# ChenRocks/UNITER

Measured on NVIDIA H100. Metric: uniter_base_encoder_fwd_bwd_samples_per_sec, higher is better.
Workload: dtype bf16

## Files before the change

uniter_b200/csrc/attn.cu:

```cuda
#include "common.h"
#include "ptx.cuh"
#include "wgmma.cuh"

namespace ub {

constexpr int ATT_D = 64;
constexpr int ATT_BM = 128;
constexpr int ATT_BN = 128;
constexpr int ATT_TILE = ATT_BM * ATT_D * 2;
constexpr int ATT_MAXSEQ = 512;
constexpr int ATT_THREADS = 256;

struct AttnParams {
  const int* cu_seqlens;
  int B, H, nheads, T;
  void* ctx;
  float* lse;
  float scale;
  uint32_t drop_thr16;
  float drop_inv_keep;
  uint32_t seed_lo, seed_hi, stream_lo, stream_hi;
  const void* dctx;
  void* dqkv;
  float* dbias;
  const unsigned long long* rng_dev;
};


__device__ __forceinline__ void frag_colsum64_atomic(const float (&d)[32], bool ok0, bool ok1, float* dst,
                                                     int lane) {
#pragma unroll
  for (int jj = 0; jj < 8; ++jj) {
#pragma unroll
    for (int t = 0; t < 2; ++t) {
      float x = (ok0 ? d[4 * jj + t] : 0.f) + (ok1 ? d[4 * jj + 2 + t] : 0.f);
      x += __shfl_xor_sync(0xffffffffu, x, 4);
      x += __shfl_xor_sync(0xffffffffu, x, 8);
      x += __shfl_xor_sync(0xffffffffu, x, 16);
      if (lane < 4) atomicAdd(dst + 8 * jj + 2 * lane + t, x);
    }
  }
}

__device__ __forceinline__ void frag_colsum64_warp(const float (&d)[32], bool ok0, bool ok1, float* dst, int lane) {
#pragma unroll
  for (int jj = 0; jj < 8; ++jj) {
#pragma unroll
    for (int t = 0; t < 2; ++t) {
      float x = (ok0 ? d[4 * jj + t] : 0.f) + (ok1 ? d[4 * jj + 2 + t] : 0.f);
      x += __shfl_xor_sync(0xffffffffu, x, 4);
      x += __shfl_xor_sync(0xffffffffu, x, 8);
      x += __shfl_xor_sync(0xffffffffu, x, 16);
      if (lane < 4) dst[8 * jj + 2 * lane + t] += x;
    }
  }
}

template <bool kBF16>
__device__ __forceinline__ void store_frag_row(void* out_row, const float (&d)[32], int e, int q4, float mul) {
  uint32_t* o = reinterpret_cast<uint32_t*>(out_row);
#pragma unroll
  for (int jj = 0; jj < 8; ++jj)
    o[(8 * jj + 2 * q4) >> 1] = Elem<kBF16>::pack(d[4 * jj + 2 * e] * mul, d[4 * jj + 2 * e + 1] * mul);
}

__device__ __forceinline__ uint64_t attn_drop_group(int bh, int q, int key8) {
  return ((static_cast<uint64_t>(bh) * ATT_MAXSEQ + q) * ATT_MAXSEQ + key8) >> 3;
}

__device__ __forceinline__ void quad_drop_words(const DropoutRng& rng, int bh, int q, int key_base, int jb,
                                                int lane, uint32_t (&w)[4]) {
  const int q4 = lane & 3;
  const uint4 r = rng.draw8(attn_drop_group(bh, q, key_base + 8 * (4 * jb + q4)));
  uint32_t got[4];
#pragma unroll
  for (int k = 0; k < 4; ++k) {
    const int sw = (q4 - k) & 3;
    const uint32_t v = sw == 0 ? r.x : (sw == 1 ? r.y : (sw == 2 ? r.z : r.w));
    got[k] = __shfl_sync(0xffffffffu, v, (lane & ~3) | ((q4 + k) & 3));
  }
#pragma unroll
  for (int t = 0; t < 4; ++t) {
    const int k = (t - q4) & 3;
    w[t] = k == 0 ? got[0] : (k == 1 ? got[1] : (k == 2 ? got[2] : got[3]));
  }
}

__device__ __forceinline__ uint32_t rand16_half(uint32_t w, int t) { return t ? (w >> 16) : (w & 0xFFFFu); }

__device__ __forceinline__ void st_swz128_u32(uint8_t* base, int r, int col, uint32_t v) {
  const int slab = col >> 6;
  const int chunk = (col & 63) >> 3;
  uint8_t* p = base + slab * ATT_TILE + r * 128 + ((chunk ^ (r & 7)) << 4) + (col & 7) * 2;
  *reinterpret_cast<uint32_t*>(p) = v;
}

template <bool kBF16>
__device__ __forceinline__ void row_delta_lse(const AttnParams& p, int seq0, int head, int row, bool ok, int q4,
                                              float& delta, float& lse2) {
  using T16 = typename Elem<kBF16>::T;
  float d = 0.f;
  lse2 = 0.f;
  if (ok) {
    const size_t off = static_cast<size_t>(seq0 + row) * p.H + head * ATT_D + 16 * q4;
    const uint4* g_do = reinterpret_cast<const uint4*>(reinterpret_cast<const T16*>(p.dctx) + off);
    const uint4* g_o = reinterpret_cast<const uint4*>(reinterpret_cast<const T16*>(p.ctx) + off);
#pragma unroll
    for (int v = 0; v < 2; ++v) {
      const uint4 a = __ldg(g_do + v), o = __ldg(g_o + v);
      float2 x, y;
      x = Elem<kBF16>::unpack(a.x); y = Elem<kBF16>::unpack(o.x); d += x.x * y.x + x.y * y.y;
      x = Elem<kBF16>::unpack(a.y); y = Elem<kBF16>::unpack(o.y); d += x.x * y.x + x.y * y.y;
      x = Elem<kBF16>::unpack(a.z); y = Elem<kBF16>::unpack(o.z); d += x.x * y.x + x.y * y.y;
      x = Elem<kBF16>::unpack(a.w); y = Elem<kBF16>::unpack(o.w); d += x.x * y.x + x.y * y.y;
    }
    lse2 = p.lse[static_cast<size_t>(head) * p.T + seq0 + row] * 1.4426950408889634f;
  }
  d += __shfl_xor_sync(0xffffffffu, d, 1);
  d += __shfl_xor_sync(0xffffffffu, d, 2);
  delta = d;
}

constexpr int SH_TILE = 64 * ATT_D * 2;
constexpr int SH_THREADS = 128;
constexpr int SH_MAXSEQ = 128;

__device__ __forceinline__ void wg_sync() { asm volatile("bar.sync 1, 128;" ::: "memory"); }

__device__ __forceinline__ int seq_blocks(const int* cu, int b) { return min((cu[b + 1] - cu[b] + 63) >> 6, 2); }

struct ShortSched {
  const int* cu;
  int B, nheads, h, b;
  long long start, hi;

  __device__ bool valid() const { return h < nheads && start < hi; }
  __device__ int blocks() const { return seq_blocks(cu, b); }

  __device__ void init(const int* cu_, int B_, int nheads_, int lane) {
    cu = cu_; B = B_; nheads = nheads_;
    h = nheads; start = hi = 0;
    int wb = 0;
    for (int b0 = 0; b0 < B; b0 += 32) {
      int c = b0 + lane < B ? seq_blocks(cu, b0 + lane) : 0;
      c *= c;
#pragma unroll
      for (int d = 16; d >= 1; d >>= 1) c += __shfl_xor_sync(0xffffffffu, c, d);
      wb += c;
    }
    if (wb == 0) return;
    const long long W = static_cast<long long>(nheads) * wb;
    const long long lo = W * blockIdx.x / gridDim.x;
    hi = W * (blockIdx.x + 1) / gridDim.x;
    if (lo >= hi) return;
    const int hh = static_cast<int>(lo / wb);
    const long long r = lo - static_cast<long long>(hh) * wb;
    int pref = 0;
    for (int b0 = 0; b0 < B; b0 += 32) {
      int c = b0 + lane < B ? seq_blocks(cu, b0 + lane) : 0;
      c *= c;
      int incl = c;
#pragma unroll
      for (int d = 1; d < 32; d <<= 1) {
        const int t = __shfl_up_sync(0xffffffffu, incl, d);
        if (lane >= d) incl += t;
      }
      const int excl = pref + incl - c;
      const unsigned m = __ballot_sync(0xffffffffu, b0 + lane < B && excl >= r);
      if (m) {
        const int L = __ffs(m) - 1;
        h = hh;
        b = b0 + L;
        start = static_cast<long long>(hh) * wb + __shfl_sync(0xffffffffu, excl, L);
        skip_empty();
        return;
      }
      pref += __shfl_sync(0xffffffffu, incl, 31);
    }
    h = hh + 1;
    b = 0;
    start = static_cast<long long>(h) * wb;
    skip_empty();
  }
  __device__ void step() {
    const int nb = blocks();
    start += nb * nb;
    if (++b == B) { b = 0; ++h; }
  }
  __device__ void skip_empty() {
    while (valid() && cu[b + 1] == cu[b]) step();
  }
  __device__ void next() { step(); skip_empty(); }
};

template <bool kBF16, int NB>
__device__ __forceinline__ void attn_fwd_short_rows(const AttnParams& p, uint32_t uQ, uint32_t uK, uint32_t uV,
                                                    int qb, int S, int seq0, int head, int bh,
                                                    const DropoutRng& rng, int warp, int lane) {
  const int q4 = lane & 3;
  const float c = p.scale * 1.4426950408889634f;
  int qrow[2];
#pragma unroll
  for (int e = 0; e < 2; ++e) qrow[e] = 64 * qb + 16 * warp + (lane >> 2) + 8 * e;

  float s[NB][32];
  wgmma_fence();
#pragma unroll
  for (int kb = 0; kb < NB; ++kb)
#pragma unroll
    for (int k = 0; k < ATT_D / 16; ++k)
      Wgmma<64, kBF16, 0, 0>::ss(s[kb], gmma_desc(uQ + qb * SH_TILE + k * 32, 16, 1024),
                                 gmma_desc(uK + kb * SH_TILE + k * 32, 16, 1024), k != 0);
  wgmma_commit();
  wgmma_wait<0>();

  float m[2] = {-INFINITY, -INFINITY}, l[2] = {0.f, 0.f};
#pragma unroll
  for (int kb = 0; kb < NB; ++kb)
#pragma unroll
    for (int i = 0; i < 32; ++i) {
      const int key = 64 * kb + 8 * (i >> 2) + 2 * q4 + (i & 1);
      if (key < S) m[(i >> 1) & 1] = fmaxf(m[(i >> 1) & 1], s[kb][i]);
    }
#pragma unroll
  for (int e = 0; e < 2; ++e) {
    m[e] = fmaxf(m[e], __shfl_xor_sync(0xffffffffu, m[e], 1));
    m[e] = fmaxf(m[e], __shfl_xor_sync(0xffffffffu, m[e], 2));
  }
  const float mc[2] = {m[0] * c, m[1] * c};

#pragma unroll
  for (int kb = 0; kb < NB; ++kb) {
#pragma unroll
    for (int jb = 0; jb < 2; ++jb) {
      uint32_t dw[2][4];
#pragma unroll
      for (int e = 0; e < 2; ++e)
        if (p.drop_thr16) quad_drop_words(rng, bh, qrow[e], 64 * kb, jb, lane, dw[e]);
#pragma unroll
      for (int jq = 0; jq < 4; ++jq) {
        const int jj = 4 * jb + jq;
#pragma unroll
        for (int e = 0; e < 2; ++e) {
#pragma unroll
          for (int t = 0; t < 2; ++t) {
            const int i = 4 * jj + 2 * e + t;
            const int key = 64 * kb + 8 * jj + 2 * q4 + t;
            float pv = key < S ? ex2_approx(fmaf(s[kb][i], c, -mc[e])) : 0.f;
            l[e] += pv;
            if (p.drop_thr16) {
              const float pr = Elem<kBF16>::to_f(Elem<kBF16>::from_f(pv));
              pv = (rand16_half(dw[e][jq], t) < p.drop_thr16) ? 0.f : pr * p.drop_inv_keep;
            }
            s[kb][i] = pv;
          }
        }
      }
    }
  }

  float o[32];
  wgmma_fence();
#pragma unroll
  for (int kb = 0; kb < NB; ++kb)
#pragma unroll
    for (int kk = 0; kk < 4; ++kk) {
      const uint32_t a[4] = {Elem<kBF16>::pack(s[kb][8 * kk + 0], s[kb][8 * kk + 1]),
                             Elem<kBF16>::pack(s[kb][8 * kk + 2], s[kb][8 * kk + 3]),
                             Elem<kBF16>::pack(s[kb][8 * kk + 4], s[kb][8 * kk + 5]),
                             Elem<kBF16>::pack(s[kb][8 * kk + 6], s[kb][8 * kk + 7])};
      Wgmma<64, kBF16, 0, 1>::rs(o, a, gmma_desc(uV + kb * SH_TILE + kk * 2048, 8192, 1024), (kb | kk) != 0);
    }
  wgmma_commit();
  wgmma_wait<0>();

#pragma unroll
  for (int e = 0; e < 2; ++e) {
    l[e] += __shfl_xor_sync(0xffffffffu, l[e], 1);
    l[e] += __shfl_xor_sync(0xffffffffu, l[e], 2);
    if (qrow[e] >= S) continue;
    if (q4 == 0) p.lse[static_cast<size_t>(head) * p.T + seq0 + qrow[e]] = m[e] * p.scale + logf(l[e]);
    typename Elem<kBF16>::T* out = reinterpret_cast<typename Elem<kBF16>::T*>(p.ctx) +
                                   static_cast<size_t>(seq0 + qrow[e]) * p.H + head * ATT_D;
    store_frag_row<kBF16>(out, o, e, q4, 1.f / l[e]);
  }
}

template <bool kBF16>
__global__ void __launch_bounds__(SH_THREADS, 2)
attn_fwd_short_kernel(const __grid_constant__ CUtensorMap tmQKV64, const AttnParams p) {
  pdl_launch_dependents();
  pdl_wait();
  extern __shared__ __align__(1024) uint8_t smem_raw[];
  uint8_t* smem = smem_raw + ((1024u - (smem_u32(smem_raw) & 1023u)) & 1023u);
  uint8_t* sQ = smem;
  uint8_t* sK = smem + 2 * SH_TILE;
  uint8_t* sV = smem + 4 * SH_TILE;
  uint64_t* bar = reinterpret_cast<uint64_t*>(smem + 6 * SH_TILE);

  const int tid = threadIdx.x, warp = tid >> 5, lane = tid & 31;
  if (tid == 0) {
    tma_prefetch_desc(&tmQKV64);
    mbar_init(&bar[0], 1);
    mbar_init(&bar[1], 1);
    fence_barrier_init();
  }
  wg_sync();
  uint32_t rs0 = p.stream_lo, rs1 = p.stream_hi;
  if (p.drop_thr16) rng_add_dev_offset(p.rng_dev, rs0, rs1);
  DropoutRng rng;
  rng.k0 = p.seed_lo; rng.k1 = p.seed_hi; rng.s0 = rs0; rng.s1 = rs1;

  auto load = [&](const ShortSched& it, int slot) {
    const int seq0 = p.cu_seqlens[it.b], nb = it.blocks(), col = it.h * ATT_D;
    mbar_expect_tx(&bar[slot], nb * 3 * SH_TILE);
    for (int r = 0; r < nb; ++r) {
      const int o = (slot + r) * SH_TILE;
      tma_load_2d(sQ + o, &tmQKV64, &bar[slot], col, seq0 + 64 * r);
      tma_load_2d(sK + o, &tmQKV64, &bar[slot], p.H + col, seq0 + 64 * r);
      tma_load_2d(sV + o, &tmQKV64, &bar[slot], 2 * p.H + col, seq0 + 64 * r);
    }
  };

  ShortSched it;
  it.init(p.cu_seqlens, p.B, p.nheads, lane);
  if (it.valid() && tid == 0) load(it, 0);
  int slot = 0;
  uint32_t ph = 0;
  while (it.valid()) {
    ShortSched nx = it;
    nx.next();
    const int seq0 = p.cu_seqlens[it.b], S = p.cu_seqlens[it.b + 1] - seq0, nb = it.blocks();
    const bool pre = nx.valid() && nb == 1 && nx.blocks() == 1;
    const int nslot = pre ? slot ^ 1 : 0;
    if (pre && tid == 0) load(nx, nslot);
    mbar_wait(&bar[slot], (ph >> slot) & 1);
    ph ^= 1u << slot;
    const uint32_t uQ = smem_u32(sQ + slot * SH_TILE), uK = smem_u32(sK + slot * SH_TILE),
                   uV = smem_u32(sV + slot * SH_TILE);
    const int bh = it.b * p.nheads + it.h;
    if (nb == 1) {
      attn_fwd_short_rows<kBF16, 1>(p, uQ, uK, uV, 0, S, seq0, it.h, bh, rng, warp, lane);
    } else {
#pragma unroll 1
      for (int qb = 0; qb < 2; ++qb)
        attn_fwd_short_rows<kBF16, 2>(p, uQ, uK, uV, qb, S, seq0, it.h, bh, rng, warp, lane);
    }
    wg_sync();
    if (nx.valid() && !pre && tid == 0) load(nx, 0);
    it = nx;
    slot = nslot;
  }
}

constexpr int SH_FWD_SMEM = 6 * SH_TILE + 16 + 1024;

template <bool kBF16, int NB>
__device__ __forceinline__ void dq_block(float (&dq)[32], uint32_t uDS, uint32_t uK, int qb) {
  wgmma_fence();
#pragma unroll
  for (int kk = 0; kk < 4 * NB; ++kk)
    Wgmma<64, kBF16, 0, 1>::ss(dq, gmma_desc(uDS + (qb * NB + (kk >> 2)) * SH_TILE + (kk & 3) * 32, 16, 1024),
                               gmma_desc(uK + kk * 2048, 8192, 1024), kk != 0);
  wgmma_commit();
  wgmma_wait<0>();
}

template <bool kBF16, bool kBias = true>
__global__ void __launch_bounds__(SH_THREADS, 2)
attn_bwd_short_kernel(const __grid_constant__ CUtensorMap tmQKV64, const __grid_constant__ CUtensorMap tmDO64,
                      const AttnParams p) {
  using T16 = typename Elem<kBF16>::T;
  pdl_launch_dependents();
  pdl_wait();
  extern __shared__ __align__(1024) uint8_t smem_raw[];
  __shared__ float sBias[4][3 * ATT_D];
  uint8_t* smem = smem_raw + ((1024u - (smem_u32(smem_raw) & 1023u)) & 1023u);
  uint8_t* sQ = smem;
  uint8_t* sK = smem + 2 * SH_TILE;
  uint8_t* sV = smem + 4 * SH_TILE;
  uint8_t* sdO = smem + 6 * SH_TILE;
  uint8_t* sP = smem + 8 * SH_TILE;
  uint8_t* sDS = smem + 9 * SH_TILE;
  uint64_t* bar = reinterpret_cast<uint64_t*>(smem + 13 * SH_TILE);

  const int tid = threadIdx.x, warp = tid >> 5, lane = tid & 31, q4 = lane & 3;
  if (tid == 0) {
    tma_prefetch_desc(&tmQKV64);
    tma_prefetch_desc(&tmDO64);
    mbar_init(&bar[0], 1);
    mbar_init(&bar[1], 1);
    fence_barrier_init();
  }
  for (int i = tid; i < 4 * 3 * ATT_D; i += SH_THREADS) (&sBias[0][0])[i] = 0.f;
  wg_sync();
  uint32_t rs0 = p.stream_lo, rs1 = p.stream_hi;
  if (p.drop_thr16) rng_add_dev_offset(p.rng_dev, rs0, rs1);
  DropoutRng rng;
  rng.k0 = p.seed_lo; rng.k1 = p.seed_hi; rng.s0 = rs0; rng.s1 = rs1;
  const float c = p.scale * 1.4426950408889634f;
  int r_loc[2];
#pragma unroll
  for (int e = 0; e < 2; ++e) r_loc[e] = 16 * warp + (lane >> 2) + 8 * e;
  const uint32_t uP = smem_u32(sP), uDS = smem_u32(sDS);

  auto load = [&](const ShortSched& it, int slot) {
    const int seq0 = p.cu_seqlens[it.b], nb = it.blocks(), col = it.h * ATT_D;
    mbar_expect_tx(&bar[slot], nb * 4 * SH_TILE);
    for (int r = 0; r < nb; ++r) {
      const int o = (slot + r) * SH_TILE;
      tma_load_2d(sQ + o, &tmQKV64, &bar[slot], col, seq0 + 64 * r);
      tma_load_2d(sK + o, &tmQKV64, &bar[slot], p.H + col, seq0 + 64 * r);
      tma_load_2d(sV + o, &tmQKV64, &bar[slot], 2 * p.H + col, seq0 + 64 * r);
      tma_load_2d(sdO + o, &tmDO64, &bar[slot], col, seq0 + 64 * r);
    }
  };

  ShortSched it;
  it.init(p.cu_seqlens, p.B, p.nheads, lane);
  if (it.valid() && tid == 0) load(it, 0);
  int slot = 0;
  uint32_t ph = 0;
  while (it.valid()) {
    ShortSched nx = it;
    nx.next();
    const int seq0 = p.cu_seqlens[it.b], S = p.cu_seqlens[it.b + 1] - seq0, nb = it.blocks();
    const int head = it.h, bh = it.b * p.nheads + head;
    const bool pre = nx.valid() && nb == 1 && nx.blocks() == 1;
    const int nslot = pre ? slot ^ 1 : 0;
    if (pre && tid == 0) load(nx, nslot);
    mbar_wait(&bar[slot], (ph >> slot) & 1);
    ph ^= 1u << slot;
    const uint32_t uQ = smem_u32(sQ + slot * SH_TILE), udO = smem_u32(sdO + slot * SH_TILE),
                   uK = smem_u32(sK + slot * SH_TILE), uV = smem_u32(sV + slot * SH_TILE);

    for (int kb = 0; kb < nb; ++kb) {
      float dv[32], dk[32];
      for (int qb = 0; qb < nb; ++qb) {
        int qrow[2];
        bool q_ok[2];
        float delta[2], lse2[2];
#pragma unroll
        for (int e = 0; e < 2; ++e) {
          qrow[e] = 64 * qb + r_loc[e];
          q_ok[e] = qrow[e] < S;
          row_delta_lse<kBF16>(p, seq0, head, qrow[e], q_ok[e], q4, delta[e], lse2[e]);
        }
        float s[32], dp[32];
        wgmma_fence();
#pragma unroll
        for (int k = 0; k < ATT_D / 16; ++k)
          Wgmma<64, kBF16, 0, 0>::ss(s, gmma_desc(uQ + qb * SH_TILE + k * 32, 16, 1024),
                                     gmma_desc(uK + kb * SH_TILE + k * 32, 16, 1024), k != 0);
#pragma unroll
        for (int k = 0; k < ATT_D / 16; ++k)
          Wgmma<64, kBF16, 0, 0>::ss(dp, gmma_desc(udO + qb * SH_TILE + k * 32, 16, 1024),
                                     gmma_desc(uV + kb * SH_TILE + k * 32, 16, 1024), k != 0);
        wgmma_commit();
        wgmma_wait<0>();

        uint8_t* dsTile = sDS + (qb * nb + kb) * SH_TILE;
#pragma unroll
        for (int jb = 0; jb < 2; ++jb) {
          uint32_t dw[2][4];
#pragma unroll
          for (int e = 0; e < 2; ++e)
            if (p.drop_thr16) quad_drop_words(rng, bh, qrow[e], 64 * kb, jb, lane, dw[e]);
#pragma unroll
          for (int jq = 0; jq < 4; ++jq) {
            const int jj = 4 * jb + jq;
#pragma unroll
            for (int e = 0; e < 2; ++e) {
              float pd[2], ds[2];
#pragma unroll
              for (int t = 0; t < 2; ++t) {
                const int idx = 4 * jj + 2 * e + t;
                const bool ok = q_ok[e] && 64 * kb + 8 * jj + 2 * q4 + t < S;
                float pr = ok ? ex2_approx(fmaf(s[idx], c, -lse2[e])) : 0.f;
                pr = Elem<kBF16>::to_f(Elem<kBF16>::from_f(pr));
                float dpv = dp[idx];
                float pdv = pr;
                if (p.drop_thr16) {
                  const bool drop = rand16_half(dw[e][jq], t) < p.drop_thr16;
                  pdv = drop ? 0.f : pr * p.drop_inv_keep;
                  dpv = drop ? 0.f : dpv * p.drop_inv_keep;
                }
                pd[t] = pdv;
                ds[t] = ok ? pr * (dpv - delta[e]) * p.scale : 0.f;
              }
              st_swz128_u32(sP, r_loc[e], 8 * jj + 2 * q4, Elem<kBF16>::pack(pd[0], pd[1]));
              st_swz128_u32(dsTile, r_loc[e], 8 * jj + 2 * q4, Elem<kBF16>::pack(ds[0], ds[1]));
            }
          }
        }
        fence_proxy_async_smem();
        wg_sync();

        const uint32_t uDSt = smem_u32(dsTile);
        wgmma_fence();
#pragma unroll
        for (int kk = 0; kk < 4; ++kk)
          Wgmma<64, kBF16, 1, 1>::ss(dv, gmma_desc(uP + kk * 2048, SH_TILE, 1024),
                                     gmma_desc(udO + qb * SH_TILE + kk * 2048, 8192, 1024), (qb | kk) != 0);
#pragma unroll
        for (int kk = 0; kk < 4; ++kk)
          Wgmma<64, kBF16, 1, 1>::ss(dk, gmma_desc(uDSt + kk * 2048, SH_TILE, 1024),
                                     gmma_desc(uQ + qb * SH_TILE + kk * 2048, 8192, 1024), (qb | kk) != 0);
        wgmma_commit();
        wgmma_wait<0>();
        wg_sync();
      }
      int key[2];
      bool k_ok[2];
#pragma unroll
      for (int e = 0; e < 2; ++e) {
        key[e] = 64 * kb + r_loc[e];
        k_ok[e] = key[e] < S;
      }
      if (kBias && p.dbias) {
        frag_colsum64_warp(dk, k_ok[0], k_ok[1], sBias[warp] + ATT_D, lane);
        frag_colsum64_warp(dv, k_ok[0], k_ok[1], sBias[warp] + 2 * ATT_D, lane);
      }
#pragma unroll
      for (int e = 0; e < 2; ++e) {
        if (!k_ok[e]) continue;
        T16* outk = reinterpret_cast<T16*>(p.dqkv) + static_cast<size_t>(seq0 + key[e]) * (3 * p.H) + p.H +
                    head * ATT_D;
        store_frag_row<kBF16>(outk, dk, e, q4, 1.f);
        store_frag_row<kBF16>(outk + p.H, dv, e, q4, 1.f);
      }
    }

    for (int qb = 0; qb < nb; ++qb) {
      float dq[32];
      if (nb == 1) dq_block<kBF16, 1>(dq, uDS, uK, 0);
      else dq_block<kBF16, 2>(dq, uDS, uK, qb);
      bool q_ok[2];
#pragma unroll
      for (int e = 0; e < 2; ++e) q_ok[e] = 64 * qb + r_loc[e] < S;
      if (kBias && p.dbias) frag_colsum64_warp(dq, q_ok[0], q_ok[1], sBias[warp], lane);
#pragma unroll
      for (int e = 0; e < 2; ++e)
        if (q_ok[e])
          store_frag_row<kBF16>(reinterpret_cast<T16*>(p.dqkv) + static_cast<size_t>(seq0 + 64 * qb + r_loc[e]) *
                                                                       (3 * p.H) + head * ATT_D,
                                dq, e, q4, 1.f);
    }
    wg_sync();
    if (nx.valid() && !pre && tid == 0) load(nx, 0);
    if (kBias && p.dbias && (!nx.valid() || nx.h != head)) {
      for (int i = tid; i < 3 * ATT_D; i += SH_THREADS) {
        atomicAdd(p.dbias + (i >> 6) * p.H + head * ATT_D + (i & 63),
                  (sBias[0][i] + sBias[1][i]) + (sBias[2][i] + sBias[3][i]));
        sBias[0][i] = sBias[1][i] = sBias[2][i] = sBias[3][i] = 0.f;
      }
    }
    it = nx;
    slot = nslot;
  }
}

constexpr int SH_BWD_SMEM = 13 * SH_TILE + 16 + 1024;

template <bool kBF16>
__device__ __forceinline__ void qk_block(float (&s)[64], uint32_t sA, uint32_t sB, int wg) {
#pragma unroll
  for (int k = 0; k < ATT_D / 16; ++k)
    Wgmma<128, kBF16, 0, 0>::ss(s, gmma_desc(sA + wg * (64 * 128) + k * 32, 16, 1024),
                                gmma_desc(sB + k * 32, 16, 1024), k != 0);
}

template <bool kBF16>
__global__ void __launch_bounds__(ATT_THREADS, 1)
attn_fwd_kernel(const __grid_constant__ CUtensorMap tmQKV, const AttnParams p) {
  pdl_launch_dependents();
  pdl_wait();
  const int b = blockIdx.z, qt = blockIdx.x;
  const int seq0 = p.cu_seqlens[b];
  const int S = p.cu_seqlens[b + 1] - seq0;
  if (qt * ATT_BM >= S) return;
  const int head = blockIdx.y;
  const int nkv = (S + ATT_BN - 1) / ATT_BN;
  uint32_t rs0 = p.stream_lo, rs1 = p.stream_hi;
  if (p.drop_thr16) rng_add_dev_offset(p.rng_dev, rs0, rs1);

  extern __shared__ __align__(1024) uint8_t smem_raw[];
  uint8_t* smem = smem_raw + ((1024u - (smem_u32(smem_raw) & 1023u)) & 1023u);
  uint8_t* sQ = smem;
  uint8_t* sK = smem + ATT_TILE;
  uint8_t* sV = smem + 2 * ATT_TILE;
  uint64_t* bar_load = reinterpret_cast<uint64_t*>(smem + 3 * ATT_TILE);

  const int tid = threadIdx.x, warp = tid >> 5, lane = tid & 31;
  const int wg = warp >> 2, q4 = lane & 3;
  if (tid == 0) {
    tma_prefetch_desc(&tmQKV);
    mbar_init(bar_load, 1);
    fence_barrier_init();
  }
  __syncthreads();

  int qrow[2];
  bool q_ok[2];
#pragma unroll
  for (int e = 0; e < 2; ++e) {
    qrow[e] = qt * ATT_BM + 64 * wg + 16 * (warp & 3) + (lane >> 2) + 8 * e;
    q_ok[e] = qrow[e] < S;
  }
  const int bh = b * p.nheads + head;
  const float c = p.scale * 1.4426950408889634f;
  const uint32_t uQ = smem_u32(sQ), uK = smem_u32(sK), uV = smem_u32(sV);
  uint32_t ph_load = 0;
  float s[64];

  float m[2] = {-INFINITY, -INFINITY}, l[2] = {0.f, 0.f};
  for (int j = 0; j < nkv; ++j) {
    const int kv_len = min(ATT_BN, S - j * ATT_BN);
    if (tid == 0) {
      const bool with_v = (nkv == 1);
      mbar_expect_tx(bar_load, (j == 0 ? ATT_TILE : 0) + ATT_TILE + (with_v ? ATT_TILE : 0));
      if (j == 0) tma_load_2d(sQ, &tmQKV, bar_load, head * ATT_D, seq0 + qt * ATT_BM);
      tma_load_2d(sK, &tmQKV, bar_load, p.H + head * ATT_D, seq0 + j * ATT_BN);
      if (with_v) tma_load_2d(sV, &tmQKV, bar_load, 2 * p.H + head * ATT_D, seq0 + j * ATT_BN);
    }
    mbar_wait(bar_load, ph_load);
    ph_load ^= 1;
    wgmma_fence();
    qk_block<kBF16>(s, uQ, uK, wg);
    wgmma_commit();
    wgmma_wait<0>();
#pragma unroll
    for (int i = 0; i < 64; ++i) {
      const int key = 8 * (i >> 2) + 2 * q4 + (i & 1);
      if (key < kv_len) m[(i >> 1) & 1] = fmaxf(m[(i >> 1) & 1], s[i]);
    }
    if (nkv > 1) __syncthreads();
  }
#pragma unroll
  for (int e = 0; e < 2; ++e) {
    m[e] = fmaxf(m[e], __shfl_xor_sync(0xffffffffu, m[e], 1));
    m[e] = fmaxf(m[e], __shfl_xor_sync(0xffffffffu, m[e], 2));
  }
  const float mc[2] = {m[0] * c, m[1] * c};

  float o[32];
#pragma unroll
  for (int i = 0; i < 32; ++i) o[i] = 0.f;
  for (int j = 0; j < nkv; ++j) {
    const int kv_len = min(ATT_BN, S - j * ATT_BN);
    if (nkv > 1) {
      if (tid == 0) {
        mbar_expect_tx(bar_load, 2 * ATT_TILE);
        tma_load_2d(sK, &tmQKV, bar_load, p.H + head * ATT_D, seq0 + j * ATT_BN);
        tma_load_2d(sV, &tmQKV, bar_load, 2 * p.H + head * ATT_D, seq0 + j * ATT_BN);
      }
      mbar_wait(bar_load, ph_load);
      ph_load ^= 1;
      wgmma_fence();
      qk_block<kBF16>(s, uQ, uK, wg);
      wgmma_commit();
      wgmma_wait<0>();
    }
    DropoutRng rng;
    rng.k0 = p.seed_lo; rng.k1 = p.seed_hi; rng.s0 = rs0; rng.s1 = rs1;
#pragma unroll
    for (int jb = 0; jb < 4; ++jb) {
      uint32_t dw[2][4];
#pragma unroll
      for (int e = 0; e < 2; ++e)
        if (p.drop_thr16) quad_drop_words(rng, bh, qrow[e], j * ATT_BN, jb, lane, dw[e]);
#pragma unroll
      for (int jq = 0; jq < 4; ++jq) {
        const int jj = 4 * jb + jq;
#pragma unroll
        for (int e = 0; e < 2; ++e) {
#pragma unroll
          for (int t = 0; t < 2; ++t) {
            const int i = 4 * jj + 2 * e + t;
            const int key = 8 * jj + 2 * q4 + t;
            float pv = key < kv_len ? ex2_approx(fmaf(s[i], c, -mc[e])) : 0.f;
            l[e] += pv;
            if (p.drop_thr16) {
              const float pr = Elem<kBF16>::to_f(Elem<kBF16>::from_f(pv));
              pv = (rand16_half(dw[e][jq], t) < p.drop_thr16) ? 0.f : pr * p.drop_inv_keep;
            }
            s[i] = pv;
          }
        }
      }
    }
    wgmma_fence();
#pragma unroll
    for (int kk = 0; kk < ATT_BN / 16; ++kk) {
      const uint32_t a[4] = {Elem<kBF16>::pack(s[8 * kk + 0], s[8 * kk + 1]),
                             Elem<kBF16>::pack(s[8 * kk + 2], s[8 * kk + 3]),
                             Elem<kBF16>::pack(s[8 * kk + 4], s[8 * kk + 5]),
                             Elem<kBF16>::pack(s[8 * kk + 6], s[8 * kk + 7])};
      Wgmma<64, kBF16, 0, 1>::rs(o, a, gmma_desc(uV + kk * 2048, 8192, 1024), (j | kk) != 0);
    }
    wgmma_commit();
    wgmma_wait<0>();
    if (nkv > 1) __syncthreads();
  }

#pragma unroll
  for (int e = 0; e < 2; ++e) {
    l[e] += __shfl_xor_sync(0xffffffffu, l[e], 1);
    l[e] += __shfl_xor_sync(0xffffffffu, l[e], 2);
    if (!q_ok[e]) continue;
    if (q4 == 0) p.lse[static_cast<size_t>(head) * p.T + seq0 + qrow[e]] = m[e] * p.scale + logf(l[e]);
    typename Elem<kBF16>::T* out = reinterpret_cast<typename Elem<kBF16>::T*>(p.ctx) +
                                   static_cast<size_t>(seq0 + qrow[e]) * p.H + head * ATT_D;
    store_frag_row<kBF16>(out, o, e, q4, 1.f / l[e]);
  }
}

constexpr int ATT_FWD_SMEM = 3 * ATT_TILE + 64 + 1024;

template <bool kBF16>
__global__ void __launch_bounds__(ATT_THREADS, 1)
attn_bwd_kernel(const __grid_constant__ CUtensorMap tmQKV, const __grid_constant__ CUtensorMap tmDO,
                const AttnParams p, float* dq_accum) {
  using T16 = typename Elem<kBF16>::T;
  pdl_launch_dependents();
  pdl_wait();
  const int b = blockIdx.z, j = blockIdx.x;
  const int seq0 = p.cu_seqlens[b];
  const int S = p.cu_seqlens[b + 1] - seq0;
  if (j * ATT_BN >= S) return;
  const int head = blockIdx.y;
  const int nq = (S + ATT_BM - 1) / ATT_BM;
  const int nkv = (S + ATT_BN - 1) / ATT_BN;
  uint32_t rs0 = p.stream_lo, rs1 = p.stream_hi;
  if (p.drop_thr16) rng_add_dev_offset(p.rng_dev, rs0, rs1);
  const int kv_len = min(ATT_BN, S - j * ATT_BN);

  extern __shared__ __align__(1024) uint8_t smem_raw[];
  uint8_t* smem = smem_raw + ((1024u - (smem_u32(smem_raw) & 1023u)) & 1023u);
  uint8_t* sQ = smem;
  uint8_t* sdO = smem + ATT_TILE;
  uint8_t* sK = smem + 2 * ATT_TILE;
  uint8_t* sV = smem + 3 * ATT_TILE;
  uint8_t* sP = smem + 4 * ATT_TILE;
  uint8_t* sDS = smem + 6 * ATT_TILE;
  uint64_t* bar_load = reinterpret_cast<uint64_t*>(smem + 8 * ATT_TILE);

  const int tid = threadIdx.x, warp = tid >> 5, lane = tid & 31;
  const int wg = warp >> 2, q4 = lane & 3;
  if (tid == 0) {
    tma_prefetch_desc(&tmQKV);
    tma_prefetch_desc(&tmDO);
    mbar_init(bar_load, 1);
    fence_barrier_init();
  }
  __syncthreads();
  int r_loc[2];
#pragma unroll
  for (int e = 0; e < 2; ++e) r_loc[e] = 64 * wg + 16 * (warp & 3) + (lane >> 2) + 8 * e;
  const int bh = b * p.nheads + head;
  const float c = p.scale * 1.4426950408889634f;
  const uint32_t uQ = smem_u32(sQ), udO = smem_u32(sdO), uK = smem_u32(sK), uV = smem_u32(sV);
  const uint32_t uP = smem_u32(sP), uDS = smem_u32(sDS);
  uint32_t ph_load = 0;
  float dv[32], dk[32];
#pragma unroll
  for (int i = 0; i < 32; ++i) { dv[i] = 0.f; dk[i] = 0.f; }

  for (int i = 0; i < nq; ++i) {
    int qrow[2];
    bool q_ok[2];
#pragma unroll
    for (int e = 0; e < 2; ++e) {
      qrow[e] = i * ATT_BM + r_loc[e];
      q_ok[e] = qrow[e] < S;
    }
    if (tid == 0) {
      mbar_expect_tx(bar_load, (i == 0 ? 4 : 2) * ATT_TILE);
      tma_load_2d(sQ, &tmQKV, bar_load, head * ATT_D, seq0 + i * ATT_BM);
      tma_load_2d(sdO, &tmDO, bar_load, head * ATT_D, seq0 + i * ATT_BM);
      if (i == 0) {
        tma_load_2d(sK, &tmQKV, bar_load, p.H + head * ATT_D, seq0 + j * ATT_BN);
        tma_load_2d(sV, &tmQKV, bar_load, 2 * p.H + head * ATT_D, seq0 + j * ATT_BN);
      }
    }

    float delta[2], lse2[2];
#pragma unroll
    for (int e = 0; e < 2; ++e) row_delta_lse<kBF16>(p, seq0, head, qrow[e], q_ok[e], q4, delta[e], lse2[e]);

    mbar_wait(bar_load, ph_load);
    ph_load ^= 1;
    float s[64], dp[64];
    wgmma_fence();
    qk_block<kBF16>(s, uQ, uK, wg);
    qk_block<kBF16>(dp, udO, uV, wg);
    wgmma_commit();
    wgmma_wait<0>();

    DropoutRng rng;
    rng.k0 = p.seed_lo; rng.k1 = p.seed_hi; rng.s0 = rs0; rng.s1 = rs1;
#pragma unroll
    for (int jb = 0; jb < 4; ++jb) {
      uint32_t dw[2][4];
#pragma unroll
      for (int e = 0; e < 2; ++e)
        if (p.drop_thr16) quad_drop_words(rng, bh, qrow[e], j * ATT_BN, jb, lane, dw[e]);
#pragma unroll
      for (int jq = 0; jq < 4; ++jq) {
        const int jj = 4 * jb + jq;
#pragma unroll
        for (int e = 0; e < 2; ++e) {
          float pd[2], ds[2];
#pragma unroll
          for (int t = 0; t < 2; ++t) {
            const int idx = 4 * jj + 2 * e + t;
            const int key = 8 * jj + 2 * q4 + t;
            const bool ok = q_ok[e] && key < kv_len;
            float pr = ok ? ex2_approx(fmaf(s[idx], c, -lse2[e])) : 0.f;
            pr = Elem<kBF16>::to_f(Elem<kBF16>::from_f(pr));
            float dpv = dp[idx];
            float pdv = pr;
            if (p.drop_thr16) {
              const bool drop = rand16_half(dw[e][jq], t) < p.drop_thr16;
              pdv = drop ? 0.f : pr * p.drop_inv_keep;
              dpv = drop ? 0.f : dpv * p.drop_inv_keep;
            }
            pd[t] = pdv;
            ds[t] = ok ? pr * (dpv - delta[e]) * p.scale : 0.f;
          }
          st_swz128_u32(sP, r_loc[e], 8 * jj + 2 * q4, Elem<kBF16>::pack(pd[0], pd[1]));
          st_swz128_u32(sDS, r_loc[e], 8 * jj + 2 * q4, Elem<kBF16>::pack(ds[0], ds[1]));
        }
      }
    }
    fence_proxy_async_smem();
    __syncthreads();

    float dq[32];
    wgmma_fence();
#pragma unroll
    for (int kk = 0; kk < ATT_BM / 16; ++kk)
      Wgmma<64, kBF16, 1, 1>::ss(dv, gmma_desc(uP + wg * ATT_TILE + kk * 2048, ATT_TILE, 1024),
                                 gmma_desc(udO + kk * 2048, 8192, 1024), (i | kk) != 0);
#pragma unroll
    for (int kk = 0; kk < ATT_BM / 16; ++kk)
      Wgmma<64, kBF16, 1, 1>::ss(dk, gmma_desc(uDS + wg * ATT_TILE + kk * 2048, ATT_TILE, 1024),
                                 gmma_desc(uQ + kk * 2048, 8192, 1024), (i | kk) != 0);
#pragma unroll
    for (int kk = 0; kk < ATT_BN / 16; ++kk)
      Wgmma<64, kBF16, 0, 1>::ss(dq, gmma_desc(uDS + (kk >> 2) * ATT_TILE + wg * (64 * 128) + (kk & 3) * 32, 16, 1024),
                                 gmma_desc(uK + kk * 2048, 8192, 1024), kk != 0);
    wgmma_commit();
    wgmma_wait<0>();
    if (p.dbias)
      frag_colsum64_atomic(dq, q_ok[0], q_ok[1], p.dbias + head * ATT_D, lane);
#pragma unroll
    for (int e = 0; e < 2; ++e) {
      if (!q_ok[e]) continue;
      if (nkv == 1) {
        store_frag_row<kBF16>(reinterpret_cast<T16*>(p.dqkv) + static_cast<size_t>(seq0 + qrow[e]) * (3 * p.H) +
                                  head * ATT_D, dq, e, q4, 1.f);
      } else {
        float* acc = dq_accum + static_cast<size_t>(seq0 + qrow[e]) * p.H + head * ATT_D;
#pragma unroll
        for (int jj = 0; jj < 8; ++jj) {
          atomicAdd(acc + 8 * jj + 2 * q4, dq[4 * jj + 2 * e]);
          atomicAdd(acc + 8 * jj + 2 * q4 + 1, dq[4 * jj + 2 * e + 1]);
        }
      }
    }
    if (i + 1 < nq) __syncthreads();
  }

  int key[2];
  bool k_ok[2];
#pragma unroll
  for (int e = 0; e < 2; ++e) {
    key[e] = j * ATT_BN + r_loc[e];
    k_ok[e] = key[e] < S;
  }
  if (p.dbias) {
    frag_colsum64_atomic(dk, k_ok[0], k_ok[1], p.dbias + p.H + head * ATT_D, lane);
    frag_colsum64_atomic(dv, k_ok[0], k_ok[1], p.dbias + 2 * p.H + head * ATT_D, lane);
  }
#pragma unroll
  for (int e = 0; e < 2; ++e) {
    if (!k_ok[e]) continue;
    T16* outk = reinterpret_cast<T16*>(p.dqkv) + static_cast<size_t>(seq0 + key[e]) * (3 * p.H) + p.H +
                head * ATT_D;
    store_frag_row<kBF16>(outk, dk, e, q4, 1.f);
    store_frag_row<kBF16>(outk + p.H, dv, e, q4, 1.f);
  }
}

template <bool kBF16>
__global__ void attn_dq_convert_kernel(const float* __restrict__ acc, void* dqkv,
                                       const int* __restrict__ cu_seqlens, int H) {
  pdl_launch_dependents();
  pdl_wait();
  const int seq0 = cu_seqlens[blockIdx.x];
  const int S = cu_seqlens[blockIdx.x + 1] - seq0;
  if (S <= ATT_BN) return;
  const int nvec = S * H / 8;
  for (int v = threadIdx.x; v < nvec; v += blockDim.x) {
    const int row = (v * 8) / H, col = (v * 8) % H;
    const float* src = acc + static_cast<size_t>(seq0 + row) * H + col;
    const float4 a = *reinterpret_cast<const float4*>(src);
    const float4 b = *reinterpret_cast<const float4*>(src + 4);
    uint4 u;
    u.x = Elem<kBF16>::pack(a.x, a.y); u.y = Elem<kBF16>::pack(a.z, a.w);
    u.z = Elem<kBF16>::pack(b.x, b.y); u.w = Elem<kBF16>::pack(b.z, b.w);
    *reinterpret_cast<uint4*>(reinterpret_cast<typename Elem<kBF16>::T*>(dqkv) +
                              static_cast<size_t>(seq0 + row) * 3 * H + col) = u;
  }
}

constexpr int ATT_BWD_SMEM = 8 * ATT_TILE + 64 + 1024;

static AttnParams attn_params(const ub200_attn_args& a) {
  AttnParams p{};
  p.cu_seqlens = a.cu_seqlens;
  p.B = a.batch; p.H = a.hidden; p.nheads = a.num_heads; p.T = a.total_tokens;
  p.ctx = a.ctx; p.lse = a.lse;
  p.scale = 0.125f;
  if (a.dropout_p > 0.f) {
    const DropoutThreshold d = dropout_threshold(a.dropout_p);
    p.drop_thr16 = d.thr16;
    p.drop_inv_keep = d.inv_keep;
  } else {
    p.drop_thr16 = 0; p.drop_inv_keep = 1.f;
  }
  p.seed_lo = static_cast<uint32_t>(a.rng_seed); p.seed_hi = static_cast<uint32_t>(a.rng_seed >> 32);
  p.stream_lo = static_cast<uint32_t>(a.rng_stream);
  p.stream_hi = static_cast<uint32_t>(a.rng_stream >> 32);
  p.rng_dev = reinterpret_cast<const unsigned long long*>(a.rng_offset_dev);
  return p;
}

static dim3 short_grid(const ub200_attn_args& a, int per_sm) {
  const long long items = static_cast<long long>(a.batch) * a.num_heads;
  const long long g = static_cast<long long>(num_sms()) * per_sm;
  return dim3(static_cast<unsigned>(g < items ? g : items));
}

}

extern "C" int ub200_attn_fwd(const ub200_attn_args* args, ub200_stream_t stream_) {
  using namespace ub;
  UB_CHECK_ARG(args != nullptr, "attn_fwd: args is NULL");
  const ub200_attn_args& a = *args;
  cudaStream_t stream = reinterpret_cast<cudaStream_t>(stream_);
  UB_CHECK_ARG(a.qkv && a.ctx && a.lse && a.cu_seqlens, "attn_fwd: null pointer");
  UB_CHECK_ARG(a.batch > 0 && a.total_tokens > 0, "attn_fwd: empty batch");
  UB_CHECK_ARG(a.num_heads > 0 && a.hidden == a.num_heads * ATT_D,
               "attn_fwd: head_dim must be 64 (hidden=%d heads=%d)", a.hidden, a.num_heads);
  UB_CHECK_ARG(a.max_seqlen > 0 && a.max_seqlen <= ATT_MAXSEQ,
               "attn_fwd: max_seqlen %d outside (0, %d]", a.max_seqlen, ATT_MAXSEQ);
  UB_CHECK_ARG(a.dtype == UB200_F16 || a.dtype == UB200_BF16, "attn_fwd: bad dtype");
  UB_CHECK_ARG(a.dropout_p >= 0.f && a.dropout_p < 1.f, "attn_fwd: dropout_p out of range");

  const AttnParams p = attn_params(a);
  const bool bf = a.dtype == UB200_BF16;
  CUtensorMap tm;
  if (a.max_seqlen <= SH_MAXSEQ) {
    int rc = make_tma_2d(&tm, a.qkv, a.dtype, a.total_tokens, 3 * a.hidden, 3 * a.hidden, 64, ATT_D);
    if (rc) return rc;
    void (*kern)(const CUtensorMap, const AttnParams) = bf ? attn_fwd_short_kernel<true> : attn_fwd_short_kernel<false>;
    static unsigned long long configured[2] = {0, 0};
    if (first_use_on_device(configured[bf ? 1 : 0]))
      UB_CHECK_CUDA(cudaFuncSetAttribute(kern, cudaFuncAttributeMaxDynamicSharedMemorySize, SH_FWD_SMEM));
    ProfScope ps(stream);
    UB_CHECK_CUDA(launch_pdl(kern, short_grid(a, 2), dim3(SH_THREADS), SH_FWD_SMEM, stream, 1, tm, p));
  } else {
    int rc = make_tma_2d(&tm, a.qkv, a.dtype, a.total_tokens, 3 * a.hidden, 3 * a.hidden, ATT_BM, ATT_D);
    if (rc) return rc;
    dim3 grid((a.max_seqlen + ATT_BM - 1) / ATT_BM, a.num_heads, a.batch);
    void (*kern)(const CUtensorMap, const AttnParams) = bf ? attn_fwd_kernel<true> : attn_fwd_kernel<false>;
    static unsigned long long configured[2] = {0, 0};
    if (first_use_on_device(configured[bf ? 1 : 0]))
      UB_CHECK_CUDA(cudaFuncSetAttribute(kern, cudaFuncAttributeMaxDynamicSharedMemorySize, ATT_FWD_SMEM));
    ProfScope ps(stream);
    UB_CHECK_CUDA(launch_pdl(kern, grid, dim3(ATT_THREADS), ATT_FWD_SMEM, stream, 1, tm, p));
  }
  UB_CHECK_CUDA(cudaGetLastError());
  return 0;
}

extern "C" int64_t ub200_attn_bwd_workspace_bytes(int32_t total_tokens, int32_t hidden,
                                                  int32_t max_seqlen) {
  if (max_seqlen <= ub::ATT_BN) return 0;
  return static_cast<int64_t>(total_tokens) * hidden * 4;
}

extern "C" int ub200_attn_bwd(const ub200_attn_args* args, ub200_stream_t stream_) {
  using namespace ub;
  UB_CHECK_ARG(args != nullptr, "attn_bwd: args is NULL");
  const ub200_attn_args& a = *args;
  cudaStream_t stream = reinterpret_cast<cudaStream_t>(stream_);
  UB_CHECK_ARG(a.qkv && a.ctx && a.lse && a.cu_seqlens && a.dctx && a.dqkv, "attn_bwd: null pointer");
  UB_CHECK_ARG(a.batch > 0 && a.total_tokens > 0, "attn_bwd: empty batch");
  UB_CHECK_ARG(a.num_heads > 0 && a.hidden == a.num_heads * ATT_D, "attn_bwd: head_dim must be 64");
  UB_CHECK_ARG(a.max_seqlen > 0 && a.max_seqlen <= ATT_MAXSEQ, "attn_bwd: max_seqlen %d outside (0, %d]",
               a.max_seqlen, ATT_MAXSEQ);
  UB_CHECK_ARG(a.dtype == UB200_F16 || a.dtype == UB200_BF16, "attn_bwd: bad dtype");
  const bool multi = a.max_seqlen > ATT_BN;
  UB_CHECK_ARG(!multi || a.workspace, "attn_bwd: max_seqlen > 128 needs the dQ workspace");

  AttnParams p = attn_params(a);
  p.dctx = a.dctx; p.dqkv = a.dqkv; p.dbias = a.dbias;
  const int di = a.dtype == UB200_BF16 ? 1 : 0;

  if (deterministic()) {
    if (a.max_seqlen > SH_MAXSEQ)
      return set_error(UB200_EUNSUPPORTED, "attn_bwd: deterministic mode supports max_seqlen <= %d (got %d)",
                       SH_MAXSEQ, a.max_seqlen);
    CUtensorMap tmQ, tmD;
    int rc = make_tma_2d(&tmQ, a.qkv, a.dtype, a.total_tokens, 3 * a.hidden, 3 * a.hidden, 64, ATT_D);
    if (rc) return rc;
    rc = make_tma_2d(&tmD, a.dctx, a.dtype, a.total_tokens, a.hidden, a.hidden, 64, ATT_D);
    if (rc) return rc;
    p.dbias = nullptr;
    void (*kern)(const CUtensorMap, const CUtensorMap, const AttnParams) =
        di ? attn_bwd_short_kernel<true, false> : attn_bwd_short_kernel<false, false>;
    static unsigned long long configured[2] = {0, 0};
    if (first_use_on_device(configured[di]))
      UB_CHECK_CUDA(cudaFuncSetAttribute(kern, cudaFuncAttributeMaxDynamicSharedMemorySize, SH_BWD_SMEM));
    {
      ProfScope ps(stream);
      UB_CHECK_CUDA(launch_pdl(kern, short_grid(a, 2), dim3(SH_THREADS), SH_BWD_SMEM, stream, 1, tmQ, tmD, p));
    }
    UB_CHECK_CUDA(cudaGetLastError());
    if (a.dbias)
      return launch_colsum_det(a.dtype, a.dqkv, a.dbias, a.total_tokens, 3 * a.hidden, 3 * a.hidden, stream,
                               a.cu_seqlens + a.batch);
    return 0;
  }

  if (a.max_seqlen <= SH_MAXSEQ) {
    CUtensorMap tmQ, tmD;
    int rc = make_tma_2d(&tmQ, a.qkv, a.dtype, a.total_tokens, 3 * a.hidden, 3 * a.hidden, 64, ATT_D);
    if (rc) return rc;
    rc = make_tma_2d(&tmD, a.dctx, a.dtype, a.total_tokens, a.hidden, a.hidden, 64, ATT_D);
    if (rc) return rc;
    void (*kern)(const CUtensorMap, const CUtensorMap, const AttnParams) =
        di ? attn_bwd_short_kernel<true> : attn_bwd_short_kernel<false>;
    static unsigned long long configured[2] = {0, 0};
    if (first_use_on_device(configured[di]))
      UB_CHECK_CUDA(cudaFuncSetAttribute(kern, cudaFuncAttributeMaxDynamicSharedMemorySize, SH_BWD_SMEM));
    ProfScope ps(stream);
    UB_CHECK_CUDA(launch_pdl(kern, short_grid(a, 2), dim3(SH_THREADS), SH_BWD_SMEM, stream, 1, tmQ, tmD, p));
    UB_CHECK_CUDA(cudaGetLastError());
    return 0;
  }

  CUtensorMap tmQ, tmD;
  int rc = make_tma_2d(&tmQ, a.qkv, a.dtype, a.total_tokens, 3 * a.hidden, 3 * a.hidden, ATT_BM, ATT_D);
  if (rc) return rc;
  rc = make_tma_2d(&tmD, a.dctx, a.dtype, a.total_tokens, a.hidden, a.hidden, ATT_BM, ATT_D);
  if (rc) return rc;
  float* acc = reinterpret_cast<float*>(a.workspace);
  UB_CHECK_CUDA(cudaMemsetAsync(acc, 0, static_cast<size_t>(a.total_tokens) * a.hidden * 4, stream));

  dim3 grid((a.max_seqlen + ATT_BN - 1) / ATT_BN, a.num_heads, a.batch);
  void (*kern)(const CUtensorMap, const CUtensorMap, const AttnParams, float*) =
      di ? attn_bwd_kernel<true> : attn_bwd_kernel<false>;
  static unsigned long long configured[2] = {0, 0};
  if (first_use_on_device(configured[di]))
    UB_CHECK_CUDA(cudaFuncSetAttribute(kern, cudaFuncAttributeMaxDynamicSharedMemorySize, ATT_BWD_SMEM));
  {
    ProfScope ps(stream);
    UB_CHECK_CUDA(launch_pdl(kern, grid, dim3(ATT_THREADS), ATT_BWD_SMEM, stream, 1, tmQ, tmD, p, acc));
  }
  UB_CHECK_CUDA(cudaGetLastError());
  {
    ProfScope ps(stream);
    if (di) UB_CHECK_CUDA(launch_pdl(attn_dq_convert_kernel<true>, dim3(a.batch), dim3(256), 0, stream, 1, static_cast<const float*>(acc), a.dqkv, a.cu_seqlens, a.hidden));
    else UB_CHECK_CUDA(launch_pdl(attn_dq_convert_kernel<false>, dim3(a.batch), dim3(256), 0, stream, 1, static_cast<const float*>(acc), a.dqkv, a.cu_seqlens, a.hidden));
    UB_CHECK_CUDA(cudaGetLastError());
  }
  return 0;
}
```

Baseline: 11270.

## Warp-specialize short attention forward with TMA producer and three consumer warpgroups

Restructures the short-sequence attention forward kernel into a producer warpgroup issuing TMA loads into a 4-slot full/empty mbarrier ring and three consumer warpgroups that take query blocks by static least-loaded assignment. Registers are rebalanced with setmaxnreg, the kernel runs one CTA per SM, and the P operand fragments are packed before the wgmma chain. The aim is to hide load latency behind compute and raise tensor-core utilization, at the cost of more shared memory, possible load imbalance, and register-pressure risk at 160 registers per consumer. The forward attention is only part of the full encoder fwd+bwd step.

```diff
diff --git a/uniter_b200/csrc/attn.cu b/uniter_b200/csrc/attn.cu
--- a/uniter_b200/csrc/attn.cu
+++ b/uniter_b200/csrc/attn.cu
@@ -259,18 +259,21 @@
     }
   }
 
+  uint32_t a[NB][4][4];
+#pragma unroll
+  for (int kb = 0; kb < NB; ++kb)
+#pragma unroll
+    for (int kk = 0; kk < 4; ++kk)
+#pragma unroll
+      for (int r = 0; r < 4; ++r) a[kb][kk][r] = Elem<kBF16>::pack(s[kb][8 * kk + 2 * r], s[kb][8 * kk + 2 * r + 1]);
   float o[32];
   wgmma_fence();
 #pragma unroll
   for (int kb = 0; kb < NB; ++kb)
 #pragma unroll
-    for (int kk = 0; kk < 4; ++kk) {
-      const uint32_t a[4] = {Elem<kBF16>::pack(s[kb][8 * kk + 0], s[kb][8 * kk + 1]),
-                             Elem<kBF16>::pack(s[kb][8 * kk + 2], s[kb][8 * kk + 3]),
-                             Elem<kBF16>::pack(s[kb][8 * kk + 4], s[kb][8 * kk + 5]),
-                             Elem<kBF16>::pack(s[kb][8 * kk + 6], s[kb][8 * kk + 7])};
-      Wgmma<64, kBF16, 0, 1>::rs(o, a, gmma_desc(uV + kb * SH_TILE + kk * 2048, 8192, 1024), (kb | kk) != 0);
-    }
+    for (int kk = 0; kk < 4; ++kk)
+      Wgmma<64, kBF16, 0, 1>::rs(o, a[kb][kk], gmma_desc(uV + kb * SH_TILE + kk * 2048, 8192, 1024),
+                                 (kb | kk) != 0);
   wgmma_commit();
   wgmma_wait<0>();
 
@@ -286,74 +289,93 @@
   }
 }
 
+constexpr int SHF_CONSUMERS = 3;
+constexpr int SHF_THREADS = 128 * (SHF_CONSUMERS + 1);
+constexpr int SHF_SLOTS = 4;
+constexpr int SHF_SLOT_BYTES = 6 * SH_TILE;
+constexpr int SHF_PRODUCER_REGS = 32;
+constexpr int SHF_CONSUMER_REGS = 160;
+
+__device__ __forceinline__ void mbar_arrive_cnt(uint64_t* bar, uint32_t count) {
+  asm volatile("mbarrier.arrive.shared::cta.b64 _, [%0], %1;" ::"r"(smem_u32(bar)), "r"(count) : "memory");
+}
+
+template <int N>
+__device__ __forceinline__ void setmaxnreg_dec() { asm volatile("setmaxnreg.dec.sync.aligned.u32 %0;" ::"n"(N) : "memory"); }
+template <int N>
+__device__ __forceinline__ void setmaxnreg_inc() { asm volatile("setmaxnreg.inc.sync.aligned.u32 %0;" ::"n"(N) : "memory"); }
+
 template <bool kBF16>
-__global__ void __launch_bounds__(SH_THREADS, 2)
+__global__ void __launch_bounds__(SHF_THREADS, 1)
 attn_fwd_short_kernel(const __grid_constant__ CUtensorMap tmQKV64, const AttnParams p) {
   pdl_launch_dependents();
   pdl_wait();
   extern __shared__ __align__(1024) uint8_t smem_raw[];
   uint8_t* smem = smem_raw + ((1024u - (smem_u32(smem_raw) & 1023u)) & 1023u);
-  uint8_t* sQ = smem;
-  uint8_t* sK = smem + 2 * SH_TILE;
-  uint8_t* sV = smem + 4 * SH_TILE;
-  uint64_t* bar = reinterpret_cast<uint64_t*>(smem + 6 * SH_TILE);
-
-  const int tid = threadIdx.x, warp = tid >> 5, lane = tid & 31;
+  uint64_t* full = reinterpret_cast<uint64_t*>(smem + SHF_SLOTS * SHF_SLOT_BYTES);
+  uint64_t* empty = full + SHF_SLOTS;
+
+  const int tid = threadIdx.x, wg = tid >> 7, warp = (tid >> 5) & 3, lane = tid & 31;
   if (tid == 0) {
     tma_prefetch_desc(&tmQKV64);
-    mbar_init(&bar[0], 1);
-    mbar_init(&bar[1], 1);
+    for (int s = 0; s < SHF_SLOTS; ++s) {
+      mbar_init(&full[s], 1);
+      mbar_init(&empty[s], 2 * 128);
+    }
     fence_barrier_init();
   }
-  wg_sync();
+  __syncthreads();
+  ShortSched it;
+  it.init(p.cu_seqlens, p.B, p.nheads, lane);
+
+  if (wg == 0) {
+    setmaxnreg_dec<SHF_PRODUCER_REGS>();
+    if (tid != 0) return;
+    for (int i = 0; it.valid(); ++i, it.next()) {
+      const int s = i % SHF_SLOTS;
+      mbar_wait(&empty[s], ((i / SHF_SLOTS) & 1) ^ 1);
+      const int seq0 = p.cu_seqlens[it.b], nb = it.blocks(), col = it.h * ATT_D;
+      uint8_t* slot = smem + s * SHF_SLOT_BYTES;
+      mbar_expect_tx(&full[s], nb * 3 * SH_TILE);
+      for (int r = 0; r < nb; ++r) {
+        tma_load_2d(slot + r * SH_TILE, &tmQKV64, &full[s], col, seq0 + 64 * r);
+        tma_load_2d(slot + (2 + r) * SH_TILE, &tmQKV64, &full[s], p.H + col, seq0 + 64 * r);
+        tma_load_2d(slot + (4 + r) * SH_TILE, &tmQKV64, &full[s], 2 * p.H + col, seq0 + 64 * r);
+      }
+    }
+    return;
+  }
+
+  setmaxnreg_inc<SHF_CONSUMER_REGS>();
+  const int consumer = wg - 1;
   uint32_t rs0 = p.stream_lo, rs1 = p.stream_hi;
   if (p.drop_thr16) rng_add_dev_offset(p.rng_dev, rs0, rs1);
   DropoutRng rng;
   rng.k0 = p.seed_lo; rng.k1 = p.seed_hi; rng.s0 = rs0; rng.s1 = rs1;
-
-  auto load = [&](const ShortSched& it, int slot) {
-    const int seq0 = p.cu_seqlens[it.b], nb = it.blocks(), col = it.h * ATT_D;
-    mbar_expect_tx(&bar[slot], nb * 3 * SH_TILE);
-    for (int r = 0; r < nb; ++r) {
-      const int o = (slot + r) * SH_TILE;
-      tma_load_2d(sQ + o, &tmQKV64, &bar[slot], col, seq0 + 64 * r);
-      tma_load_2d(sK + o, &tmQKV64, &bar[slot], p.H + col, seq0 + 64 * r);
-      tma_load_2d(sV + o, &tmQKV64, &bar[slot], 2 * p.H + col, seq0 + 64 * r);
-    }
-  };
-
-  ShortSched it;
-  it.init(p.cu_seqlens, p.B, p.nheads, lane);
-  if (it.valid() && tid == 0) load(it, 0);
-  int slot = 0;
-  uint32_t ph = 0;
-  while (it.valid()) {
-    ShortSched nx = it;
-    nx.next();
-    const int seq0 = p.cu_seqlens[it.b], S = p.cu_seqlens[it.b + 1] - seq0, nb = it.blocks();
-    const bool pre = nx.valid() && nb == 1 && nx.blocks() == 1;
-    const int nslot = pre ? slot ^ 1 : 0;
-    if (pre && tid == 0) load(nx, nslot);
-    mbar_wait(&bar[slot], (ph >> slot) & 1);
-    ph ^= 1u << slot;
-    const uint32_t uQ = smem_u32(sQ + slot * SH_TILE), uK = smem_u32(sK + slot * SH_TILE),
-                   uV = smem_u32(sV + slot * SH_TILE);
-    const int bh = it.b * p.nheads + it.h;
-    if (nb == 1) {
-      attn_fwd_short_rows<kBF16, 1>(p, uQ, uK, uV, 0, S, seq0, it.h, bh, rng, warp, lane);
-    } else {
-#pragma unroll 1
-      for (int qb = 0; qb < 2; ++qb)
-        attn_fwd_short_rows<kBF16, 2>(p, uQ, uK, uV, qb, S, seq0, it.h, bh, rng, warp, lane);
-    }
-    wg_sync();
-    if (nx.valid() && !pre && tid == 0) load(nx, 0);
-    it = nx;
-    slot = nslot;
-  }
-}
-
-constexpr int SH_FWD_SMEM = 6 * SH_TILE + 16 + 1024;
+  int work[SHF_CONSUMERS] = {};
+  for (int i = 0; it.valid(); ++i, it.next()) {
+    const int s = i % SHF_SLOTS;
+    const int nb = it.blocks();
+    for (int qb = 0; qb < nb; ++qb) {
+      int c = 0, least = work[0];
+#pragma unroll
+      for (int k = 1; k < SHF_CONSUMERS; ++k)
+        if (work[k] < least) { c = k; least = work[k]; }
+#pragma unroll
+      for (int k = 0; k < SHF_CONSUMERS; ++k) work[k] += k == c ? nb : 0;
+      if (c != consumer) continue;
+      const int seq0 = p.cu_seqlens[it.b], S = p.cu_seqlens[it.b + 1] - seq0;
+      const uint32_t uQ = smem_u32(smem + s * SHF_SLOT_BYTES), uK = uQ + 2 * SH_TILE, uV = uQ + 4 * SH_TILE;
+      const int bh = it.b * p.nheads + it.h;
+      mbar_wait(&full[s], (i / SHF_SLOTS) & 1);
+      if (nb == 1) attn_fwd_short_rows<kBF16, 1>(p, uQ, uK, uV, 0, S, seq0, it.h, bh, rng, warp, lane);
+      else attn_fwd_short_rows<kBF16, 2>(p, uQ, uK, uV, qb, S, seq0, it.h, bh, rng, warp, lane);
+      mbar_arrive_cnt(&empty[s], 2 / nb);
+    }
+  }
+}
+
+constexpr int SH_FWD_SMEM = SHF_SLOTS * SHF_SLOT_BYTES + 2 * SHF_SLOTS * 8 + 1024;
 
 template <bool kBF16, int NB>
 __device__ __forceinline__ void dq_block(float (&dq)[32], uint32_t uDS, uint32_t uK, int qb) {
@@ -970,7 +992,7 @@
     if (first_use_on_device(configured[bf ? 1 : 0]))
       UB_CHECK_CUDA(cudaFuncSetAttribute(kern, cudaFuncAttributeMaxDynamicSharedMemorySize, SH_FWD_SMEM));
     ProfScope ps(stream);
-    UB_CHECK_CUDA(launch_pdl(kern, short_grid(a, 2), dim3(SH_THREADS), SH_FWD_SMEM, stream, 1, tm, p));
+    UB_CHECK_CUDA(launch_pdl(kern, short_grid(a, 1), dim3(SHF_THREADS), SH_FWD_SMEM, stream, 1, tm, p));
   } else {
     int rc = make_tma_2d(&tm, a.qkv, a.dtype, a.total_tokens, 3 * a.hidden, 3 * a.hidden, ATT_BM, ATT_D);
     if (rc) return rc;
```

After: 11510 (median of 6 runs). 2.2% higher.
